# kjenike/panagram

Hardware: AMD Instinct MI355X
Metric: anchored k-mers/sec building pan-kmer bitmap (higher is better)
Workload: dtype u64

## Files before the change

panagram_amd/csrc/pg_anchor.hip:

```cpp
#include "pg_kernels.h"
#include <map>
#include <mutex>
#include <utility>
#include <type_traits>

#include <algorithm>

#ifndef PG_ANCHOR_PART
#define PG_ANCHOR_PART -1
#endif
#define PG_HAS_PART(n) (PG_ANCHOR_PART == -1 || PG_ANCHOR_PART == (n))
#define PG_MAIN_PART (PG_ANCHOR_PART <= 0)
#if defined(PG_PHASE_TIMING) && PG_ANCHOR_PART != -1
#error "a -DPG_PHASE_TIMING build keeps its counters in one device variable: compile pg_anchor.hip as ONE unit (PG_ANCHOR_PART unset)"
#endif

namespace pg {

hipError_t probe_part0(hipStream_t s, uint32_t w, uint32_t ntiles, const SubTable &st, const uint64_t *seqw, const uint32_t *nmw, const uint32_t *has_n,
                       const SeqDesc *sd, const AnchorDesc *ad, const uint32_t *tile_contig, const uint32_t *sched, uint32_t tile_base, uint8_t *out1,
                       uint32_t nbytes, const RowCols &rc, int rowmode, const FuseArgs *fuse);
hipError_t probe_part1(hipStream_t s, uint32_t w, uint32_t ntiles, const SubTable &st, const uint64_t *seqw, const uint32_t *nmw, const uint32_t *has_n,
                       const SeqDesc *sd, const AnchorDesc *ad, const uint32_t *tile_contig, const uint32_t *sched, uint32_t tile_base, uint8_t *out1,
                       uint32_t nbytes, const RowCols &rc, int rowmode, const FuseArgs *fuse);
hipError_t probe_part2(hipStream_t s, uint32_t w, uint32_t ntiles, const SubTable &st, const uint64_t *seqw, const uint32_t *nmw, const uint32_t *has_n,
                       const SeqDesc *sd, const AnchorDesc *ad, const uint32_t *tile_contig, const uint32_t *sched, uint32_t tile_base, uint8_t *out1,
                       uint32_t nbytes, const RowCols &rc, int rowmode, const FuseArgs *fuse);
hipError_t insert_part0(hipStream_t s, uint32_t win, uint32_t ntiles, const SubTable &st, int w, uint32_t bits, uint32_t count_mode, const uint64_t *seqw,
                        const uint32_t *nmw, const uint32_t *has_n, const SeqDesc *sd, const uint32_t *tile0, uint32_t ncontigs,
                        unsigned long long *counters, uint32_t max_probe);
hipError_t insert_part1(hipStream_t s, uint32_t win, uint32_t ntiles, const SubTable &st, int w, uint32_t bits, uint32_t count_mode, const uint64_t *seqw,
                        const uint32_t *nmw, const uint32_t *has_n, const SeqDesc *sd, const uint32_t *tile0, uint32_t ncontigs,
                        unsigned long long *counters, uint32_t max_probe);
hipError_t insert_part2(hipStream_t s, uint32_t win, uint32_t ntiles, const SubTable &st, int w, uint32_t bits, uint32_t count_mode, const uint64_t *seqw,
                        const uint32_t *nmw, const uint32_t *has_n, const SeqDesc *sd, const uint32_t *tile0, uint32_t ncontigs,
                        unsigned long long *counters, uint32_t max_probe);
hipError_t preload_part1();
hipError_t preload_part2();

constexpr int PROBE_SEQW = ((PROBE_TILE + 31) / 32 + 6 + 3) & ~3;
#ifndef PG_ABLATE
#define PG_ABLATE 0
#endif
constexpr uint32_t PROBE_SEQ_BASES = 32u * PROBE_SEQW;
#ifdef PG_PHASE_TIMING
__device__ unsigned long long pg_phase_cycles[1024 * 16];
#define PG_PH_DECL uint32_t ph_acc[12] = {0, 0, 0, 0, 0, 0, 0, 0, 0, 0, 0, 0}; uint32_t ph_t = (uint32_t)__builtin_readcyclecounter();
#define PG_PH(i) { const uint32_t ph_n = (uint32_t)__builtin_readcyclecounter(); ph_acc[i] += ph_n - ph_t; ph_t = ph_n; }
#define PG_PH_FLUSH { if (threadIdx.x == 0) { for (int ph_i = 0; ph_i < 9; ++ph_i) atomicAdd(&pg_phase_cycles[(blockIdx.x & 1023u) * 16u + ph_i], (unsigned long long)ph_acc[ph_i]); atomicAdd(&pg_phase_cycles[(blockIdx.x & 1023u) * 16u + 9], 1ull); atomicAdd(&pg_phase_cycles[(blockIdx.x & 1023u) * 16u + 10], (unsigned long long)ph_acc[10]); } }
#else
#define PG_PH_DECL
#define PG_PH(i)
#define PG_PH_FLUSH
#endif
__device__ __forceinline__ uint64_t revcomp_window(const uint64_t *rw, uint32_t p, uint64_t kmask, uint32_t rcb) {
    return extract_bases32(reinterpret_cast<const uint32_t *>(rw), rcb - p) & kmask;
}

__device__ __forceinline__ void stage_chunk(uint4 *line, uint32_t slot, int slots, const uint4 v) {
    uint2 *const p = reinterpret_cast<uint2 *>(line);
    p[slot] = make_uint2(v.x, v.y);
    p[slots + slot] = make_uint2(v.z, v.w);
}
template <bool TWO, int SLOTS>
__device__ __forceinline__ int scan_line_lds(const uint4 *line, uint64_t key, uint32_t &m0, uint32_t &m1) {
    uint64_t kk[SLOTS];
#pragma unroll
    for (int j = 0; j < SLOTS / 2; ++j) {
        const uint4 v = line[j];
        kk[2 * j] = (uint64_t)v.x | ((uint64_t)v.y << 32);
        kk[2 * j + 1] = (uint64_t)v.z | ((uint64_t)v.w << 32);
    }
    constexpr uint32_t SLOT_BYTES = 8u, MASK0 = 8u * SLOTS;
    m0 = m1 = 0;
    if constexpr (SLOTS == 8) {
        unsigned long long e[8];
#pragma unroll
        for (int sl = 0; sl < 8; ++sl) e[sl] = __builtin_amdgcn_ballot_w64(kk[sl] == key);
        const unsigned long long b0 = e[1] | e[3] | e[5] | e[7], b1 = e[2] | e[3] | e[6] | e[7], b2 = e[4] | e[5] | e[6] | e[7];
        const unsigned long long any = b0 | b1 | b2 | e[0];
        const bool hit = __builtin_amdgcn_inverse_ballot_w64(any);
#if PG_ABLATE == 6
        if (hit) m0 = (uint32_t)b0 | 1u;
        return hit ? 1 : (kk[SLOTS - 1] == EMPTY_KEY ? 0 : -1);
#elif PG_ABLATE == 7
        m0 = (uint32_t)(kk[0] ^ kk[1] ^ kk[2] ^ kk[3] ^ kk[4] ^ kk[5] ^ kk[6] ^ kk[7]) | 1u;
        return (kk[0] ^ kk[3]) == key ? -1 : 1;
#endif
        if (hit) {
            const uint32_t off = (__builtin_amdgcn_inverse_ballot_w64(b0) ? SLOT_BYTES : 0u) | (__builtin_amdgcn_inverse_ballot_w64(b1) ? 2u * SLOT_BYTES : 0u) |
                                 (__builtin_amdgcn_inverse_ballot_w64(b2) ? 4u * SLOT_BYTES : 0u);
            if constexpr (TWO) {
                const uint2 mk = *reinterpret_cast<const uint2 *>(reinterpret_cast<const uint8_t *>(line) + off + MASK0);
                m0 = mk.x;
                m1 = mk.y;
            } else {
                m0 = *reinterpret_cast<const uint32_t *>(reinterpret_cast<const uint8_t *>(line) + off + MASK0);
            }
        }
        return hit ? 1 : (kk[SLOTS - 1] == EMPTY_KEY ? 0 : -1);
    } else {
        int hit = -1;
#pragma unroll
        for (int sl = 0; sl < SLOTS; ++sl) hit = (kk[sl] == key) ? sl : hit;
        if (hit >= 0) {
            const uint2 mk = *reinterpret_cast<const uint2 *>(reinterpret_cast<const uint8_t *>(line) + (uint32_t)hit * SLOT_BYTES + MASK0);
            m0 = mk.x;
            if (TWO) m1 = mk.y;
        }
        return hit >= 0 ? 1 : (kk[SLOTS - 1] == EMPTY_KEY ? 0 : -1);
    }
}


template <bool TWO, int SLOTS>
__device__ __forceinline__ int scan_line_global(const SubTable &st, uint32_t b, uint64_t key, uint32_t &m0, uint32_t &m1) {
    const uint4 *line = reinterpret_cast<const uint4 *>(st.buckets + (uint64_t)b * (16 * SLOTS));
    uint4 v[SLOTS];
#pragma unroll
    for (int sl = 0; sl < SLOTS; ++sl) v[sl] = line[sl];
    m0 = m1 = 0;
#pragma unroll
    for (int sl = 0; sl < SLOTS; ++sl) {
        const uint64_t kk = (uint64_t)v[sl].x | ((uint64_t)v[sl].y << 32);
        const bool hit = (kk == key);
        m0 = hit ? v[sl].z : m0;
        if (TWO) m1 = hit ? v[sl].w : m1;
    }
    const uint64_t last = (uint64_t)v[SLOTS - 1].x | ((uint64_t)v[SLOTS - 1].y << 32);
    return (m0 | m1) ? 1 : (last == EMPTY_KEY ? 0 : -1);
}

template <bool TWO, int SLOTS>
__device__ __forceinline__ void lane_chase(const SubTable &st, uint64_t key, uint32_t level, uint32_t b, uint32_t step,
                                           uint32_t &m0, uint32_t &m1) {
    for (uint64_t n = 0; n < st.nbuckets + GROUP_CHAIN; ++n) {
// ... 260 lines not shown

__device__ __forceinline__ uint32_t lane_up1(uint32_t v) {
    return (uint32_t)__builtin_amdgcn_update_dpp((int)v, (int)v, 0x138 , 0xf, 0xf, false);
}
__device__ __forceinline__ unsigned long long differs_from_lane_below(uint32_t v) {
    uint32_t t;
    asm("s_nop 1\n\tv_xor_b32_dpp %0, %1, %1 wave_shr:1 row_mask:0xf bank_mask:0xf" : "=&v"(t) : "v"(v));
    return __builtin_amdgcn_ballot_w64(t != 0u);
}
#define PG_DPPMIN "s_nop 1\n\tv_min_u32_dpp %0, %0, %1 wave_shr:1 row_mask:0xf bank_mask:0xf\n\t"
template <int W>
__device__ __forceinline__ uint32_t sliding_min(uint32_t x) {
    uint32_t m = x;
    if constexpr (W == 2) asm(PG_DPPMIN : "+v"(m) : "v"(x));
    if constexpr (W == 3) asm(PG_DPPMIN PG_DPPMIN : "+v"(m) : "v"(x));
    if constexpr (W == 4) asm(PG_DPPMIN PG_DPPMIN PG_DPPMIN : "+v"(m) : "v"(x));
    if constexpr (W == 5) asm(PG_DPPMIN PG_DPPMIN PG_DPPMIN PG_DPPMIN : "+v"(m) : "v"(x));
    if constexpr (W == 6) asm(PG_DPPMIN PG_DPPMIN PG_DPPMIN PG_DPPMIN PG_DPPMIN : "+v"(m) : "v"(x));
    if constexpr (W == 7) asm(PG_DPPMIN PG_DPPMIN PG_DPPMIN PG_DPPMIN PG_DPPMIN PG_DPPMIN : "+v"(m) : "v"(x));
    if constexpr (W == 8) asm(PG_DPPMIN PG_DPPMIN PG_DPPMIN PG_DPPMIN PG_DPPMIN PG_DPPMIN PG_DPPMIN : "+v"(m) : "v"(x));
    static_assert(W >= 1 && W <= 8, "minimizer window");
    return m;
}
#undef PG_DPPMIN
__device__ __forceinline__ uint32_t suffix_min8_row(uint32_t x) {
    uint32_t r = x;
    asm("s_nop 1\n\tv_min_u32_dpp %0, %0, %0 row_shl:1 row_mask:0xf bank_mask:0xf\n\t"
        "s_nop 1\n\tv_min_u32_dpp %0, %0, %0 row_shl:2 row_mask:0xf bank_mask:0xf\n\t"
        "s_nop 1\n\tv_min_u32_dpp %0, %0, %0 row_shl:4 row_mask:0xf bank_mask:0xf"
        : "+v"(r));
    return r;
}
#define PG_F "v_min_u32_dpp %0, %0, %0 wave_shr:1 row_mask:0xf bank_mask:0xf\n\t"
#define PG_S(n) "v_min_u32_dpp %1, %1, %1 row_shl:" #n " row_mask:0xf bank_mask:0xf\n\t"
#define PG_N0 "s_nop 0\n\t"
#define PG_N1 "s_nop 1\n\t"
template <int W>
__device__ __forceinline__ uint32_t sliding_min_suffix(uint32_t x, uint32_t &suffix) {
    uint32_t m = x, r = suffix;
    static_assert(W >= 2 && W <= 8, "minimizer window");
    if constexpr (W == 2) asm(PG_N1 PG_F PG_S(1) PG_N1 PG_S(2) PG_N1 PG_S(4) : "+v"(m), "+v"(r));
    if constexpr (W == 3) asm(PG_N1 PG_F PG_S(1) PG_N0 PG_F PG_S(2) PG_N1 PG_S(4) : "+v"(m), "+v"(r));
    if constexpr (W == 4) asm(PG_N1 PG_F PG_S(1) PG_N0 PG_F PG_S(2) PG_N0 PG_F PG_S(4) : "+v"(m), "+v"(r));
    if constexpr (W == 5) asm(PG_N1 PG_F PG_S(1) PG_N0 PG_F PG_S(2) PG_N0 PG_F PG_S(4) PG_N0 PG_F : "+v"(m), "+v"(r));
    if constexpr (W == 6) asm(PG_N1 PG_F PG_S(1) PG_N0 PG_F PG_S(2) PG_N0 PG_F PG_S(4) PG_N0 PG_F PG_N1 PG_F : "+v"(m), "+v"(r));
    if constexpr (W == 7) asm(PG_N1 PG_F PG_S(1) PG_N0 PG_F PG_S(2) PG_N0 PG_F PG_S(4) PG_N0 PG_F PG_N1 PG_F PG_N1 PG_F : "+v"(m), "+v"(r));
    if constexpr (W == 8) asm(PG_N1 PG_F PG_S(1) PG_N0 PG_F PG_S(2) PG_N0 PG_F PG_S(4) PG_N0 PG_F PG_N1 PG_F PG_N1 PG_F PG_N1 PG_F : "+v"(m), "+v"(r));
    suffix = r;
    return m;
}
#undef PG_F
#undef PG_S
#undef PG_N0
#undef PG_N1
__device__ __forceinline__ uint32_t lanes_le_index(unsigned long long mask, uint32_t base) {
    const unsigned long long m1 = mask >> 1;
    const uint32_t c = base + (uint32_t)(mask & 1ull) - 1u;
    return __builtin_amdgcn_mbcnt_hi((uint32_t)(m1 >> 32), __builtin_amdgcn_mbcnt_lo((uint32_t)m1, c));
}

__device__ __forceinline__ uint32_t run_ids(unsigned long long lmask) {
    const uint32_t below = __builtin_amdgcn_mbcnt_hi((uint32_t)(lmask >> 32), __builtin_amdgcn_mbcnt_lo((uint32_t)lmask, ~0u));
    uint32_t rid;
    unsigned long long carry_out;
    asm("v_addc_co_u32_e64 %0, %1, %2, 0, %3" : "=v"(rid), "=s"(carry_out) : "v"(below), "s"(lmask));
    return rid;
}
__device__ __forceinline__ uint32_t set_lane_index(unsigned long long mask, uint32_t base) {
    return __builtin_amdgcn_mbcnt_hi((uint32_t)(mask >> 32), __builtin_amdgcn_mbcnt_lo((uint32_t)mask, base));
}

constexpr int COLS_G = 8;
constexpr uint32_t TILE_SLOTS = PROBE_TILE / 64;
static_assert(PROBE_TILE % 512 == 0, "the column kernels take a tile in units of 512 positions");
__device__ __forceinline__ void cols_or_position(unsigned long long *cols, uint32_t pl, uint32_t m0) {
    while (m0) {
        const uint32_t j = (uint32_t)__ffs((int)m0) - 1u;
        m0 &= m0 - 1u;
        atomicOr(&cols[(pl >> 6) * COLS_G + j], 1ull << (pl & 63u));
    }
}

template <bool TWO, int ROWMODE, int SLOTS, int MAXRUN, bool WIDE, int LEVELS, bool INL = false>
__device__ __forceinline__ void drain_queue(const SubTable &st, uint32_t qn, const uint64_t *sw, const uint64_t *rw, uint32_t *q_line,
                                            uint32_t *q_step, uint16_t *q_pl, uint32_t *lines_w, uint4 *buf,
                                            uint8_t *tile_rows, uint32_t nbytes, const RowCols rc, int lane) {
    const int k = (int)st.k;
    constexpr int LDS_LINE_U4 = SLOTS + 1;
    constexpr int STAGE_ITERS = (MAXRUN * SLOTS + 63) / 64;
    const uint8_t *chunk_base = st.buckets + (uint32_t)(lane % SLOTS) * 16u;
    const uint32_t lbytes = INL ? st.layout * 64u : st.slots * (WIDE ? 8u : 16u);
    static_assert(LEVELS >= 1, "k_probe's entries (home line, group) are turned into (next line, step) by level 1's staged batches");
    for (int level = 1; qn > 0; ++level) {
        __syncthreads();
        if (level > LEVELS) {
            for (uint32_t e = lane; e < qn; e += 64) {
                uint32_t m0, m1;
                const uint64_t key = canonical_from_le(extract_bases(sw, q_pl[e]), k);
                if constexpr (WIDE && INL) {
                    uint32_t rw4[4];
                    lane_chase_inl(st, key, (uint32_t)level, q_line[e], q_step[e], rw4);
                    if (rw4[0] | rw4[1] | rw4[2] | rw4[3]) store_row_regs(tile_rows + (uint64_t)q_pl[e] * nbytes, nbytes, rw4);
                } else if constexpr (WIDE) {
                    lane_chase_wide(st, key, (uint32_t)level, q_line[e], q_step[e], m0, m1);
                    if (m1) store_row_wide(st.masks, st.W, nbytes, tile_rows + (uint64_t)q_pl[e] * nbytes, m0, m1);
                } else {
                    lane_chase<TWO, SLOTS>(st, key, (uint32_t)level, q_line[e], q_step[e], m0, m1);
                    if constexpr (ROWMODE == 3) cols_or_position(reinterpret_cast<unsigned long long *>(tile_rows), q_pl[e], m0);
                    else if (m0 | m1) store_row<ROWMODE>(tile_rows + (uint64_t)q_pl[e] * nbytes, m0, m1, rc);
                }
            }
            break;
        }
        uint32_t kept = 0;
        for (uint32_t i0 = 0; i0 < qn; i0 += 64) {
            const uint32_t e = i0 + lane;
            const bool act = e < qn;
            const uint32_t ec = act ? e : qn - 1;
            uint32_t line = q_line[ec], step = q_step[ec];
            if (GROUP_CHAIN > 1 && level == 1) {
                step = step_of_group(step, st.nbuckets);
                line = next_line(line, step, st.nbuckets);
            }
            const uint32_t pl = q_pl[ec];
            const uint64_t kmask = kmer_mask(k);
            const uint64_t X = extract_bases32(reinterpret_cast<const uint32_t *>(sw), pl) & kmask;
            const uint64_t key = canonical_from_xb(X, revcomp_window(rw, pl, kmask, PROBE_SEQ_BASES - (uint32_t)k), k);
            const uint32_t prev_line = lane_up1(line);
            const bool leader = act && (lane == 0 || line != prev_line);
            const unsigned long long lmask = __builtin_amdgcn_ballot_w64(leader);
            const uint32_t rid = lanes_le_index(lmask, 0u);
            const uint32_t nruns = (uint32_t)__popcll(lmask);
            uint32_t m0 = 0, m1 = 0;
            [[maybe_unused]] uint32_t rw4[4] = {0, 0, 0, 0};
            int rcode = 0;
            const uint32_t padline = lmask ? (uint32_t)__builtin_amdgcn_readlane((int)line, __builtin_ctzll(lmask)) : 0u;
            for (uint32_t r0 = 0; r0 < nruns; r0 += MAXRUN) {
                const uint32_t nl = min((uint32_t)MAXRUN, nruns - r0);
                if (lane < MAXRUN) lines_w[lane] = padline;
                if (leader && rid - r0 < nl) lines_w[rid - r0] = line;
                __syncthreads();
                uint4 v[STAGE_ITERS];
                uint32_t ln[STAGE_ITERS];
#pragma unroll
                for (int u = 0; u < STAGE_ITERS; ++u) ln[u] = lines_w[u * (64 / SLOTS) + lane / SLOTS];
#pragma unroll
                for (int u = 0; u < STAGE_ITERS; ++u) v[u] = *reinterpret_cast<const uint4 *>(chunk_base + (uint64_t)ln[u] * lbytes);
#pragma unroll
                for (int u = 0; u < STAGE_ITERS; ++u) {
                    const uint32_t idx = u * 64 + lane;
                    if constexpr (WIDE) buf[(idx / SLOTS) * LDS_LINE_U4 + (idx % SLOTS)] = v[u];
                    else stage_chunk(buf + (idx / SLOTS) * LDS_LINE_U4, idx % SLOTS, SLOTS, v[u]);
                }
                __syncthreads();
                if (act && rid - r0 < nl) {
                    if constexpr (WIDE && INL) {
                        rcode = scan_keys_inl(buf + (rid - r0) * LDS_LINE_U4, key, st.slots, m1);
                        if (m1) masks_inl(buf + (rid - r0) * LDS_LINE_U4, st.slots, st.W, m1 - 1u, rw4);
                    } else if constexpr (WIDE) {
                        rcode = scan_keys16_lds(buf + (rid - r0) * LDS_LINE_U4, key, m1);
                        m0 = line;
                    } else {
                        rcode = scan_line_lds<TWO, SLOTS>(buf + (rid - r0) * LDS_LINE_U4, key, m0, m1);
                    }
                }
                __syncthreads();
            }
            const bool again = act && rcode < 0;
            if constexpr (WIDE && INL) {
                if (act && m1) store_row_regs(tile_rows + (uint64_t)pl * nbytes, nbytes, rw4);
            } else if constexpr (WIDE) {
                if (act && m1) store_row_wide(st.masks, st.W, nbytes, tile_rows + (uint64_t)pl * nbytes, m0, m1);
            } else {
                if constexpr (ROWMODE == 3) {
                    if (act) cols_or_position(reinterpret_cast<unsigned long long *>(tile_rows), pl, m0);
                } else {
                    if (act && (m0 | m1)) store_row<ROWMODE>(tile_rows + (uint64_t)pl * nbytes, m0, m1, rc);
                }
            }
            const unsigned long long kmask2 = __builtin_amdgcn_ballot_w64(again);
            if (again) {
                const uint32_t slot = set_lane_index(kmask2, kept);
                uint32_t nl2 = line, ns2 = step;
                if constexpr (LEVELS + 1 < (int)GROUP_CHAIN) nl2 = next_line(line, step, st.nbuckets);
                else advance_line(key, (uint32_t)level + 1, st.nbuckets, nl2, ns2);
                q_line[slot] = nl2;
                q_step[slot] = ns2;
                q_pl[slot] = (uint16_t)pl;
            }
            kept += (uint32_t)__popcll(kmask2);
            __syncthreads();
        }
        qn = kept;
    }
}

#ifndef PG_FUSE_LOAD_SC1
#define PG_FUSE_LOAD_SC1 1
#endif
typedef const __attribute__((address_space(1))) uint8_t *GlobalBytes;
template <int NW>
__device__ __forceinline__ void fuse_load_row(GlobalBytes base, uint32_t off, uint32_t (&w)[NW]) {
    GlobalBytes p = base + off;
#if PG_FUSE_LOAD_SC1
#pragma unroll
    for (int i = 0; i + 1 < NW; i += 2) {
        const unsigned long long v = __hip_atomic_load(reinterpret_cast<const __attribute__((address_space(1))) unsigned long long *>(p + 4 * i), __ATOMIC_RELAXED,
                                                       __HIP_MEMORY_SCOPE_AGENT);
        w[i] = (uint32_t)v, w[i + 1] = (uint32_t)(v >> 32);
    }
    if constexpr (NW & 1)
        w[NW - 1] = __hip_atomic_load(reinterpret_cast<const __attribute__((address_space(1))) uint32_t *>(p + 4 * (NW - 1)), __ATOMIC_RELAXED, __HIP_MEMORY_SCOPE_AGENT);
#else
    const WordsN<NW> v = *reinterpret_cast<const __attribute__((address_space(1))) WordsN<NW> *>(p);
#pragma unroll
    for (int i = 0; i < NW; ++i) w[i] = v.w[i];
#endif
}
__device__ __forceinline__ void fuse_flush_word(const uint32_t (&pl)[5], uint32_t *out16, int lane) {
    uint32_t R[16];
#pragma unroll
    for (int q = 0; q < 8; ++q) {
        uint32_t v = 0;
#pragma unroll
        for (int i = 0; i < 5; ++i) v |= ((pl[i] >> q) & 0x01010101u) << i;
        R[2 * q] = v & 0x00FF00FFu;
        R[2 * q + 1] = (v >> 8) & 0x00FF00FFu;
    }
#define PG_XCHG(HALF, BIT)                                                  \
    {                                                                       \
        const bool up = (lane & BIT) != 0;                                  \
        _Pragma("unroll") for (int i = 0; i < HALF; ++i) {                  \
            const uint32_t send = up ? R[i] : R[i + HALF];                  \
            const uint32_t keep = up ? R[i + HALF] : R[i];                  \
            R[i] = keep + (uint32_t)__shfl_xor((int)send, BIT);             \
        }                                                                   \
    }
    PG_XCHG(8, 32)
    PG_XCHG(4, 16)
    PG_XCHG(2, 8)
    PG_XCHG(1, 4)
#undef PG_XCHG
    R[0] += (uint32_t)__shfl_xor((int)R[0], 2);
    R[0] += (uint32_t)__shfl_xor((int)R[0], 1);
    if ((lane & 3) == 0) {
        const uint32_t idx = (uint32_t)lane >> 2;
        out16[(idx >> 1) + ((idx & 1u) ? 8u : 0u)] = R[0];
    }
}
template <int NWP, bool LASTPASS>
__device__ __forceinline__ void tile_statistics_pass(uint32_t *Hc, GlobalBytes rs, uint32_t npos, uint32_t nbytes, uint32_t woff,
                                                     uint32_t keep_last, uint32_t split, uint32_t N, uint32_t (&pcs)[4], uint32_t *cs_out, int lane) {
    const uint32_t N1 = N + 1u;
    uint32_t ones[NWP], twos[NWP], fours[NWP], eights[NWP], sixteens[NWP], hold4[NWP], hold8[NWP];
#pragma unroll
    for (int w = 0; w < NWP; ++w) ones[w] = twos[w] = fours[w] = eights[w] = sixteens[w] = hold4[w] = hold8[w] = 0;
    uint32_t nx[4][NWP];
    auto request = [&](int g, uint32_t (&dst)[4][NWP]) __attribute__((always_inline)) {
#pragma unroll
        for (int i = 0; i < 4; ++i) {
            const uint32_t r = (uint32_t)(4 * g + i) * 64u + (uint32_t)lane;
            fuse_load_row<NWP>(rs, min(r, npos - 1u) * nbytes + woff, dst[i]);
        }
    };
    request(0, nx);
#pragma unroll
    for (int g = 0; g < 4; ++g) {
        uint32_t rw[4][NWP];
#pragma unroll
        for (int i = 0; i < 4; ++i)
#pragma unroll
            for (int w = 0; w < NWP; ++w) rw[i][w] = nx[i][w];
        if (g < 3) request(g + 1, nx);
        uint32_t pc4 = pcs[g];
#pragma unroll
        for (int i = 0; i < 4; ++i) {
// ... 26 lines not shown
            u = twos[w] ^ c2a;
            const uint32_t c4 = (twos[w] & c2a) | (u & c2b);
            twos[w] = u ^ c2b;
            if ((g & 1) == 0) {
                hold4[w] = c4;
            } else {
                u = fours[w] ^ hold4[w];
                const uint32_t c8 = (fours[w] & hold4[w]) | (u & c4);
                fours[w] = u ^ c4;
                if (g == 1) {
                    hold8[w] = c8;
                } else {
                    u = eights[w] ^ hold8[w];
                    sixteens[w] = (eights[w] & hold8[w]) | (u & c8);
                    eights[w] = u ^ c8;
                }
            }
        }
    }
#pragma unroll
    for (int w = 0; w < NWP; ++w) {
        const uint32_t pl[5] = {ones[w], twos[w], fours[w], eights[w], sixteens[w]};
        fuse_flush_word(pl, cs_out + 16 * w, lane);
    }
}

template <int NW>
__device__ __forceinline__ void tile_statistics(uint32_t *H, const uint8_t *tile_rows, uint32_t npos, uint32_t nbytes, const AnchorDesc &a,
                                                uint32_t tile_start, uint32_t tile, const FuseArgs &fo, int lane) {
    const uint32_t N = fo.ngenomes, N1 = N + 1u, hw = fo.hw;
    const uint32_t nh = 2u * N1;
#ifdef PG_PHASE_TIMING
    uint32_t tph[5] = {0, 0, 0, 0, 0}, tph_t = (uint32_t)__builtin_readcyclecounter();
#define PG_TPH(i) { const uint32_t n_ = (uint32_t)__builtin_readcyclecounter(); tph[i] += n_ - tph_t; tph_t = n_; }
#else
#define PG_TPH(i)
#endif
    __builtin_amdgcn_s_waitcnt(0x0F70);
    __syncthreads();
    PG_TPH(0)
    const uint64_t base = reinterpret_cast<uint64_t>(tile_rows);
    GlobalBytes rs = reinterpret_cast<GlobalBytes>(((uint64_t)(uint32_t)__builtin_amdgcn_readfirstlane((int)(uint32_t)(base >> 32)) << 32) |
                                                   (uint32_t)__builtin_amdgcn_readfirstlane((int)(uint32_t)base));
    const uint32_t r100 = (100u - tile_start % 100u) % 100u + 100u * (uint32_t)lane;
    const bool want100 = fo.out100 != nullptr && r100 < npos;
    uint32_t w100[NW];
    fuse_load_row<NW>(rs, min(r100, npos - 1u) * nbytes, w100);
    for (uint32_t i = lane; i < 4u * nh; i += 64) H[i] = 0;
    const uint64_t bin_end = ((uint64_t)(tile_start / a.binlen) + 1u) * a.binlen;
    const uint32_t split = (uint32_t)min((uint64_t)npos, bin_end - tile_start);
    const uint32_t keep = (nbytes & 3u) ? ((1u << (8u * (nbytes & 3u))) - 1u) : ~0u;
    uint32_t *const Hc = H + ((uint32_t)lane & 3u) * nh;
    uint32_t *cs_out = fo.tile_cs + (uint64_t)tile * fo.csw;
    uint32_t pcs[4] = {0, 0, 0, 0};
    __syncthreads();
    PG_TPH(1)
    if constexpr (NW <= 2) {
        tile_statistics_pass<NW, true>(Hc, rs, npos, nbytes, 0u, keep, split, N, pcs, cs_out, lane);
        PG_TPH(2)
    } else {
        tile_statistics_pass<2, false>(Hc, rs, npos, nbytes, 0u, ~0u, split, N, pcs, cs_out, lane);
        PG_TPH(2)
        tile_statistics_pass<NW - 2, true>(Hc, rs, npos, nbytes, 8u, keep, split, N, pcs, cs_out + 32, lane);
    }
    if (want100) {
        uint8_t *dst = fo.out100 + a.out100_off + (uint64_t)((tile_start + r100) / 100u) * nbytes;
#pragma unroll
        for (int i = 0; i < NW; ++i)
#pragma unroll
            for (int b = 0; b < 4; ++b)
                if ((uint32_t)(4 * i + b) < nbytes) dst[4 * i + b] = (uint8_t)(w100[i] >> (8 * b));
    }
    __syncthreads();
    PG_TPH(3)
    uint32_t *th = fo.tile_hist + (uint64_t)tile * hw;
    for (uint32_t i = lane; i < hw; i += 64) {
        const uint32_t lo = H[2u * i] + H[nh + 2u * i] + H[2u * nh + 2u * i] + H[3u * nh + 2u * i];
        const uint32_t hi = H[2u * i + 1u] + H[nh + 2u * i + 1u] + H[2u * nh + 2u * i + 1u] + H[3u * nh + 2u * i + 1u];
        th[i] = lo | (hi << 16);
    }
    PG_TPH(4)
#ifdef PG_PHASE_TIMING
    if (lane == 0)
        for (int i = 0; i < 5; ++i) atomicAdd(&pg_phase_cycles[(blockIdx.x & 1023u) * 16u + 11 + i], (unsigned long long)tph[i]);
#endif
#undef PG_TPH
}

template <bool TWO, int ROWMODE, int SLOTS, bool WIDE>
constexpr bool probe_pipelined = SLOTS == 8 && !WIDE && ROWMODE != 3 && (ROWMODE == 1 || ROWMODE >= 4 || TWO);
template <int W_C, bool TWO, int ROWMODE, int SLOTS, bool M64, bool WIDE = false, bool INL = false, bool FUSE = false>
__global__ __launch_bounds__(64, ((probe_pipelined<TWO, ROWMODE, SLOTS, WIDE> || INL || FUSE) ? 8 : 1))
__attribute__((amdgpu_num_sgpr(80))) void k_probe(const SubTable st, const uint64_t *__restrict__ seqw,
                                              const uint32_t *__restrict__ nmw, const uint32_t *__restrict__ has_n,
                                              const SeqDesc *__restrict__ sd, const AnchorDesc *__restrict__ ad,
                                              const uint32_t *__restrict__ tile_contig,
                                              const uint32_t *__restrict__ sched, uint32_t tile_base,
                                              uint8_t *__restrict__ out1, uint32_t nbytes, const RowCols rc, const FuseArgs fo) {
    constexpr int LDS_LINE_U4 = SLOTS + 1;
    constexpr int MAXRUN = PROBE_MAXRUN;
    constexpr int STAGE_ITERS = (MAXRUN * SLOTS + 63) / 64;
    constexpr int BUF_U4 = ((STAGE_ITERS * 64 + SLOTS - 1) / SLOTS) * LDS_LINE_U4;
    constexpr int OFF_RW = PROBE_SEQW * 8, OFF_NW = OFF_RW + (PROBE_SEQW + 1) * 8, OFF_LW = OFF_NW + PROBE_SEQW * 4;
    constexpr int QCAP = PROBE_QCAP;
    constexpr int OFF_BUF = (OFF_LW + MAXRUN * 4 + 15) & ~15, OFF_QL = OFF_BUF + BUF_U4 * 16, OFF_QS = OFF_QL + QCAP * 4;
    constexpr int OFF_QP = OFF_QS + QCAP * 4, LDS_BYTES = OFF_QP + QCAP * 2;
    static_assert(OFF_LW <= 1020 || PROBE_TILE > 1024, "the sequence words must stay within reach of ds_read2_b32's offsets");
    __shared__ __attribute__((aligned(16))) uint8_t lds[LDS_BYTES];
    uint64_t *const sw = reinterpret_cast<uint64_t *>(lds);
    uint64_t *const rw = reinterpret_cast<uint64_t *>(lds + OFF_RW);
    uint32_t *const nw = reinterpret_cast<uint32_t *>(lds + OFF_NW);
    uint32_t(*const lines_w)[MAXRUN] = reinterpret_cast<uint32_t(*)[MAXRUN]>(lds + OFF_LW);
    uint4(*const buf)[BUF_U4] = reinterpret_cast<uint4(*)[BUF_U4]>(lds + OFF_BUF);
    uint32_t *const q_line = reinterpret_cast<uint32_t *>(lds + OFF_QL);
    uint32_t *const q_step = reinterpret_cast<uint32_t *>(lds + OFF_QS);
    uint16_t *const q_pl = reinterpret_cast<uint16_t *>(lds + OFF_QP);
    PG_PH_DECL
    const int lane = threadIdx.x;
    const int k = (int)st.k;
    if constexpr (W_C != 0) __builtin_assume(k >= 20 && k <= 32);
    const uint32_t tile = sched ? sched[blockIdx.x + tile_base] : blockIdx.x + tile_base;
    const uint32_t c = tile_contig[tile];
    const AnchorDesc a = ad[c];
    const SeqDesc s = sd[c];
    const uint32_t tile_start = (tile - a.tile0) * PROBE_TILE;
    const uint32_t npos = min((uint32_t)PROBE_TILE, a.nkmers - tile_start);
    const bool hasn = has_n[c] != 0;

    for (int i = lane; i < PROBE_SEQW; i += 64) {
        const uint64_t wi = (uint64_t)(tile_start >> 5) + i;
        const uint64_t wv = wi < s.nwords ? seqw[s.seq_off + wi] : 0ull;
        sw[i] = wv;
        rw[PROBE_SEQW - 1 - i] = pair_reverse64(~wv);
        nw[i] = (hasn && wi < s.nwords) ? nmw[s.seq_off + wi] : 0u;
    }
    if (lane == 0) rw[PROBE_SEQW] = 0;
    __syncthreads();

    const uint64_t kmask = W_C ? (((uint64_t)(k == 32 ? ~0u : ((1u << (2 * k - 32)) - 1u)) << 32) | 0xFFFFFFFFull) : kmer_mask(k);
    const uint32_t rcb = PROBE_SEQ_BASES - (uint32_t)k;
    constexpr int HALO = W_C ? W_C - 1 : 0;
    constexpr bool CARRY = W_C >= 2;
    constexpr bool CUT = W_C != 0;
    const uint32_t m = W_C ? (uint32_t)k - W_C + 1 : 0;
    const uint64_t mm64 = (m >= 32) ? ~0ull : ((1ull << (2 * (m ? m : 1))) - 1);
    __shared__ unsigned long long cols[ROWMODE == 3 ? TILE_SLOTS * COLS_G : 1];
    if constexpr (ROWMODE == 3) {
        for (uint32_t i = lane; i < TILE_SLOTS * COLS_G; i += 64) cols[i] = 0;
        __syncthreads();
    }
#if PG_ABLATE == 9 || PG_ABLATE == 10
    uint8_t *tile_rows = out1 + (uint64_t)(blockIdx.x & 255u) * PROBE_TILE * nbytes;
#else
    uint8_t *tile_rows = ROWMODE == 3 ? reinterpret_cast<uint8_t *>(cols) : out1 + a.out_off + (uint64_t)tile_start * nbytes;
#endif
    uint32_t qn = 0;

    const uint8_t *chunk_base = st.buckets + (uint32_t)(lane % SLOTS) * 16u;
    const uint32_t lbytes = INL ? st.layout * 64u : st.slots * (WIDE ? 8u : 16u);

    struct Front {
        uint64_t key;
        uint32_t grp, line, rid, nruns, padline;
        uint32_t adv;
        uint32_t ln[STAGE_ITERS];
        unsigned long long rmask, amask, lmask;
    };
// ... 217 lines not shown
        } else {
            if (ROWMODE == 6 && b0 + (uint32_t)__popcll(f.rmask) < npos) {
                const uint32_t mine = inrange ? m0 : 0u;
                const uint32_t nxt = (uint32_t)__builtin_amdgcn_update_dpp(0, (int)mine, 0x130 , 0xf, 0xf, true);
                struct __attribute__((packed)) U32 { uint32_t v; };
                if (inrange) reinterpret_cast<U32 *>(tile_rows + (uint32_t)pl * 3u)->v = (m0 & 0xFFFFFFu) | (nxt << 24);
            } else if constexpr (ROWMODE == 6) {
                const uint32_t nxt = (uint32_t)__builtin_amdgcn_update_dpp(0, (int)m0, 0x130 , 0xf, 0xf, false);
                const uint32_t o4 = (uint32_t)reinterpret_cast<uintptr_t>(tile_rows) & 3u;
                const uint32_t j = ((uint32_t)pl - o4) & 3u;
                const uint32_t lo = (nxt << 24) | (m0 & 0xFFFFFFu);
                const uint32_t dw = __builtin_amdgcn_alignbit(nxt >> 8, lo, 8u * j);
                const unsigned long long nextin = f.rmask >> 1;
                const unsigned long long dmask = f.rmask & nextin & __builtin_amdgcn_ballot_w64(j != 3u);
                const unsigned long long fmask = f.rmask & (1ull | ~nextin);
                uint8_t *row = tile_rows + (uint32_t)pl * 3u;
                if (__builtin_amdgcn_inverse_ballot_w64(dmask)) *reinterpret_cast<uint32_t *>(row + j) = dw;
                if (__builtin_amdgcn_inverse_ballot_w64(fmask)) store_row<ROWMODE>(row, m0, m1, rc);
            } else
#if PG_ABLATE == 2
            if (inrange && m0 == 0xDEADBEEFu)
#else
            if (ROWMODE == 0 && TWO && rc.words == 3u && nbytes >= 5u && b0 + (uint32_t)__popcll(f.rmask) < npos) {
                const uint32_t mine = inrange ? m0 : 0u;
                const uint32_t nxt = (uint32_t)__builtin_amdgcn_update_dpp(0, (int)mine, 0x130 , 0xf, 0xf, true);
                if (inrange) {
                    typedef uint32_t u32x2u __attribute__((ext_vector_type(2), aligned(1)));
                    const uint32_t t8 = 8u * (nbytes - 4u);
                    u32x2u q = {m0, (m1 & ((1u << t8) - 1u)) | (nxt << t8)};
                    *reinterpret_cast<u32x2u *>(tile_rows + (uint32_t)pl * nbytes) = q;
                }
            } else if (inrange)
#endif
                store_row<ROWMODE>(tile_rows + (ROWMODE == 1 ? (uint32_t)pl : ROWMODE == 4 ? (uint32_t)pl * 4u : ROWMODE == 5 ? (uint32_t)pl * 2u : ROWMODE == 6 ? (uint32_t)pl * 3u : (uint32_t)pl * nbytes), m0, m1, rc);
        }
        PG_PH(6)
    };
    constexpr bool PIPE = probe_pipelined<TWO, ROWMODE, SLOTS, WIDE>;
    constexpr int LEVELS = (W_C >= 6 && !TWO && !WIDE && PROBE_STAGED_LEVELS > 1) ? 1 : PROBE_STAGED_LEVELS;
    static_assert(QCAP >= 128, "an early drain must leave room for a batch");
    constexpr uint32_t QROOM = QCAP - 64;
    uint32_t b0 = 0;
    if constexpr (PIPE) {
        Lines L;
#pragma unroll
        for (int it = 0; it < STAGE_ITERS; ++it) L.v[it] = make_uint4(0, 0, 0, 0);
        PG_PH(0)
        carry = carry_at(0u);
        Front cur = front(0u);
        L = issue(cur, 0u);
        for (;;) {
            PG_PH(7)
            const uint32_t b1 = b0 + cur.adv;
            const bool more = b1 < npos;
            Front nxt = cur;
            __builtin_amdgcn_sched_barrier(0);
            if (more) nxt = front(b1);
            __builtin_amdgcn_sched_barrier(0);
            back(cur, L, b0, [&]() __attribute__((always_inline)) {
                if (more) L = issue(nxt, 0u);
            });
            __builtin_amdgcn_sched_barrier(0);
            b0 = b1;
            if (!more || qn > QROOM) break;
            cur = nxt;
        }
    } else {
        {
            carry = carry_at(0u);
            const Front f = front(0u);
            const Lines L = issue(f, 0u);
            back(f, L, 0u, [] {});
            b0 = f.adv;
        }
        while (b0 < npos && qn <= QROOM) {
            const Front f = front(b0);
            const Lines L = issue(f, 0u);
            back(f, L, b0, [] {});
            b0 += f.adv;
        }
    }
    PG_PH(7)
    for (;;) {
        drain_queue<TWO, ROWMODE, SLOTS, MAXRUN, WIDE, LEVELS, INL>(st, qn, sw, rw, q_line, q_step, q_pl, lines_w[0], buf[0], tile_rows, nbytes, rc, lane);
        qn = 0;
        if (b0 >= npos) break;
        __syncthreads();
        carry = carry_at(b0);
        while (b0 < npos && qn <= QROOM) {
            const Front f = front(b0);
            const Lines L = issue(f, 0u);
            back(f, L, b0, [] {});
            b0 += f.adv;
        }
    }
    PG_PH(8)
    PG_PH_FLUSH
    if constexpr (FUSE) {
        static_assert(ROWMODE != 1 && ROWMODE != 3 && LDS_BYTES >= 4 * 4 * 2 * 129, "fused statistics: rows of 2..16 bytes; four copies of 2 x 129 histogram counters in LDS");
        const AnchorDesc *ad2 = ad;
        const uint32_t *tc2 = tile_contig, *sched2 = sched;
        asm volatile("" : "+s"(ad2), "+s"(tc2), "+s"(sched2));
        const uint32_t tile2 = sched2 ? sched2[blockIdx.x + tile_base] : blockIdx.x + tile_base;
        const AnchorDesc a2 = ad2[tc2[tile2]];
        if (a2.binlen >= (uint32_t)PROBE_TILE) {
            const uint32_t ts2 = (tile2 - a2.tile0) * PROBE_TILE;
            const uint32_t np2 = min((uint32_t)PROBE_TILE, a2.nkmers - ts2);
            const uint8_t *rows2 = out1 + a2.out_off + (uint64_t)ts2 * nbytes;
            uint32_t *H = reinterpret_cast<uint32_t *>(lds);
            if constexpr (WIDE) {
                if (nbytes <= 12u) tile_statistics<3>(H, rows2, np2, nbytes, a2, ts2, tile2, fo, lane);
                else tile_statistics<4>(H, rows2, np2, nbytes, a2, ts2, tile2, fo, lane);
            } else {
                tile_statistics<TWO ? 2 : 1>(H, rows2, np2, nbytes, a2, ts2, tile2, fo, lane);
            }
        }
    }
    if constexpr (ROWMODE == 3) {
        __syncthreads();
        const uint32_t width = nbytes, trel = tile - tile_base;
        unsigned long long *dst = reinterpret_cast<unsigned long long *>(out1) + (uint64_t)trel * TILE_SLOTS * width;
        for (uint32_t i = lane; i < TILE_SLOTS * width; i += 64) dst[i] = cols[(i / width) * COLS_G + i % width];
    }
}

constexpr int INSERT_QCAP = 256;

template <bool COUNT, bool CLAIM = true>
__device__ __forceinline__ int wave_insert_batch(const SubTable &st, bool valid, uint64_t key, uint32_t grp, int w, uint32_t bits,
                                                 uint32_t max_probe, int lane) {
    const uint32_t kstride = key_stride(st), slots = st.slots;
    uint32_t b = home_of_group(grp, st.nbuckets), step = step_of_group(grp, st.nbuckets), probes = 0;
    int s = -1;
    bool done = !valid, fresh = false;
    int r = 0;
    auto shfl64 = [](uint64_t v, int src) __attribute__((always_inline)) {
        return (uint64_t)(uint32_t)__shfl((int)(uint32_t)v, src) | ((uint64_t)(uint32_t)__shfl((int)(uint32_t)(v >> 32), src) << 32);
    };
    auto resolve = [&](uint32_t sl, bool claimed) __attribute__((always_inline)) {
        uint32_t *mp = mask_ptr(st, b, sl, (uint32_t)w);
        if (COUNT) {
            if (*mp < 0xFFFFFF00u) atomicAdd(mp, bits);
        } else if (claimed) {
            *reinterpret_cast<volatile uint32_t *>(mp) = bits;
        } else {
            const uint32_t cur = *mp;
            if ((cur & bits) != bits) *reinterpret_cast<volatile uint32_t *>(mp) = cur | bits;
        }
        r = claimed ? 1 : 0;
        done = true;
    };
    while (__ballot(!done)) {
        if (!done && s >= (int)slots) {
            if (++probes >= max_probe) {
                done = true;
                r = -1;
            } else {
                advance_line(key, probes, st.nbuckets, b, step);
                s = -1;
            }
        }
        if (!done && s < 0) {
            uint8_t *base = st.buckets + (uint64_t)b * line_bytes(st);
            int hit = -1, fr = -1;
            for (uint32_t s0 = 0; s0 < slots; s0 += 8) {
                uint64_t kk[8];
#pragma unroll
// ... 2127 lines not shown
        auto flush = [&]() {
            if (acc) {
                if (is_hist) atomicAdd(&bins[key], (uint32_t)acc);
                else atomicAdd(&colsums[key], acc);
            }
            acc = 0;
        };
#pragma unroll
        for (uint32_t j = 0; j < TR_TILES; ++j) {
            const uint32_t t = t0 + j;
            if (t >= t1) break;
            const uint32_t c = tile_contig[t];
            if (c != cur_c) {
                cur_c = c;
                a = ad[c];
            }
            if (a.binlen < (uint32_t)PROBE_TILE) continue;
            const unsigned long long k2 = is_hist ? (a.bin_off + (uint64_t)(t - a.tile0) * PROBE_TILE / a.binlen + rel) * N1 + pc
                                                  : (unsigned long long)c * N + g;
            if (k2 != key) {
                flush();
                key = k2;
            }
            acc += (v[j] >> shift) & 0xFFFFu;
        }
        flush();
    }
}

hipError_t launch_tile_reduce(hipStream_t st, const FuseArgs &fo, const AnchorDesc *ad, const uint32_t *tile_contig, uint32_t ntiles,
                              uint32_t *bins, unsigned long long *colsums, uint32_t want_colsums) {
    if (ntiles == 0) return hipSuccess;
    const uint32_t nitems = 2u * (fo.ngenomes + 1u) + (want_colsums ? fo.ngenomes : 0u);
    const uint32_t per = std::max(1u, 256u / nitems), groups = (ntiles + TR_TILES - 1) / TR_TILES;
    hipLaunchKernelGGL(k_tile_reduce, dim3((groups + per - 1) / per), dim3(256), 0, st, fo, ad, tile_contig, ntiles, bins, colsums,
                       want_colsums);
    return hipGetLastError();
}

hipError_t launch_window_stats(hipStream_t st, uint32_t ngenomes, const uint8_t *rows, uint64_t nrows, uint32_t nwin,
                               uint32_t pieces, const uint64_t *starts, const uint64_t *ends, unsigned long long *hist,
                               unsigned long long *cs) {
    if (nwin == 0) return hipSuccess;
    hipLaunchKernelGGL(k_window_stats, dim3(nwin, pieces), dim3(256), (2 * ngenomes + 1) * 4, st, ngenomes, rows, nrows,
                       starts, ends, hist, cs);
    return hipGetLastError();
}

hipError_t launch_cols_extract(hipStream_t st, uint32_t ngenomes, const AnchorDesc *ad, const uint32_t *tile_contig,
                               uint32_t tile_base, uint32_t ntiles, const uint8_t *out1, uint32_t g0, uint32_t width, void *dst) {
    if (ntiles == 0 || width == 0) return hipSuccess;
    if (ngenomes <= 8 && g0 < 8)
        hipLaunchKernelGGL(k_cols_extract_b1, dim3((unsigned)(((uint64_t)ntiles + 4 * COLS_TPW - 1) / (4 * COLS_TPW))), dim3(256), 0, st, ngenomes, ad, tile_contig, tile_base,
                           ntiles, out1, g0, width, static_cast<uint8_t *>(dst));
    else
        hipLaunchKernelGGL(k_cols_extract, dim3((unsigned)(((uint64_t)ntiles * TILE_SLOTS + 3) / 4)), dim3(256), 0, st, ngenomes, ad,
                           tile_contig, tile_base, ntiles, out1, g0, width, static_cast<unsigned long long *>(dst));
    return hipGetLastError();
}

hipError_t launch_cols_merge(hipStream_t st, uint32_t ngenomes, const AnchorDesc *ad, const uint32_t *tile_contig,
                             uint32_t tile_base, uint32_t ntiles, uint8_t *out1, const void *src, uint32_t part0,
                             uint32_t nparts, uint64_t part_words, uint32_t per, uint32_t accumulate) {
    if (ntiles == 0 || per == 0 || nparts == 0) return hipSuccess;
    if (ngenomes <= 8)
        hipLaunchKernelGGL(k_cols_merge_b1, dim3((unsigned)(((uint64_t)ntiles + 4 * COLS_TPW - 1) / (4 * COLS_TPW))), dim3(256), 0, st, ngenomes, ad, tile_contig, tile_base,
                           ntiles, out1, static_cast<const uint8_t *>(src), part0, nparts, part_words * 8, per, accumulate);
    else
        hipLaunchKernelGGL(k_cols_merge, dim3((unsigned)(((uint64_t)ntiles * TILE_SLOTS + 3) / 4)), dim3(256), 0, st, ngenomes, ad,
                           tile_contig, tile_base, ntiles, out1, static_cast<const unsigned long long *>(src), part0, nparts,
                           part_words, per, accumulate);
    return hipGetLastError();
}

hipError_t launch_lowres(hipStream_t st, uint32_t ngenomes, const AnchorDesc *ad, const uint32_t *tile_contig,
                         uint32_t ntiles, const uint8_t *out1, uint8_t *outlow, uint32_t step) {
    if (ntiles == 0) return hipSuccess;
    hipLaunchKernelGGL(k_lowres, dim3(ntiles), dim3(64), 0, st, ngenomes, ad, tile_contig, out1, outlow, step);
    return hipGetLastError();
}

#ifdef PG_PHASE_TIMING
}
extern "C" int pg_debug_phase_cycles(unsigned long long *out16, int reset) {
    hipDeviceSynchronize();
    static unsigned long long all[1024 * 16];
    if (hipMemcpyFromSymbol(all, HIP_SYMBOL(pg::pg_phase_cycles), sizeof all) != hipSuccess) return -1;
    for (int i = 0; i < 16; ++i) out16[i] = 0;
    for (int b = 0; b < 1024; ++b)
        for (int i = 0; i < 16; ++i) out16[i] += all[b * 16 + i];
    if (reset) {
        for (auto &x : all) x = 0;
        if (hipMemcpyToSymbol(HIP_SYMBOL(pg::pg_phase_cycles), all, sizeof all) != hipSuccess) return -1;
    }
    return 0;
}
namespace pg {
#endif
hipError_t preload_anchor_kernels() {
    hipFuncAttributes fa;
    hipError_t e = hipFuncGetAttributes(&fa, reinterpret_cast<const void *>(k_lowres));
    if (e == hipSuccess) e = preload_part1();
    if (e == hipSuccess) e = preload_part2();
    return e;
}

hipError_t launch_insert_tiles(hipStream_t s, const SubTable &st, int w, uint32_t bits, int count_mode, const uint64_t *seqw,
                               const uint32_t *nmw, const uint32_t *has_n, const SeqDesc *sd, const uint32_t *tile0,
                               uint32_t ncontigs, uint32_t ntiles, unsigned long long *counters, uint32_t max_probe) {
    if (ntiles == 0) return hipSuccess;
    const uint32_t win = st.m ? st.k - st.m + 1 : 0;
    auto *part = (win == 0 || win == 3 || win == 4) ? insert_part0 : (win == 5 || win == 6) ? insert_part1 : (win == 7 || win == 8) ? insert_part2 : nullptr;
    if (!part) return hipErrorInvalidValue;
    return part(s, win, ntiles, st, w, bits, (uint32_t)count_mode, seqw, nmw, has_n, sd, tile0, ncontigs, counters, max_probe);
}
#endif

}
```

Baseline: 237.6 billion.

## Software-pipeline drain_queue line fetches and drop redundant barriers

Restructures drain_queue's staged levels so that, for non-wide tables, the global fetch of the next batch of bucket lines is issued before scanning the current batch staged in LDS. Two per-iteration __syncthreads are removed. The key computation now uses the caller's kmask and rcb, and run ids come from a ballot-based helper. The level loop is split into a templated first-level/later-level lambda, and phase-timing counters are widened to more slots. The risks are higher register pressure from holding prefetched lines and LDS races now that barriers are gone.

```diff
diff --git a/panagram_amd/csrc/pg_anchor.hip b/panagram_amd/csrc/pg_anchor.hip
--- a/panagram_amd/csrc/pg_anchor.hip
+++ b/panagram_amd/csrc/pg_anchor.hip
@@ -44,14 +44,21 @@
 #endif
 constexpr uint32_t PROBE_SEQ_BASES = 32u * PROBE_SEQW;
 #ifdef PG_PHASE_TIMING
-__device__ unsigned long long pg_phase_cycles[1024 * 16];
-#define PG_PH_DECL uint32_t ph_acc[12] = {0, 0, 0, 0, 0, 0, 0, 0, 0, 0, 0, 0}; uint32_t ph_t = (uint32_t)__builtin_readcyclecounter();
+constexpr uint32_t PG_PH_SLOTS = 32;
+__device__ unsigned long long pg_phase_cycles[1024 * PG_PH_SLOTS];
+#define PG_PH_DECL uint32_t ph_acc[24] = {0, 0, 0, 0, 0, 0, 0, 0, 0, 0, 0, 0, 0, 0, 0, 0, 0, 0, 0, 0, 0, 0, 0, 0}; uint32_t ph_t = (uint32_t)__builtin_readcyclecounter();
 #define PG_PH(i) { const uint32_t ph_n = (uint32_t)__builtin_readcyclecounter(); ph_acc[i] += ph_n - ph_t; ph_t = ph_n; }
-#define PG_PH_FLUSH { if (threadIdx.x == 0) { for (int ph_i = 0; ph_i < 9; ++ph_i) atomicAdd(&pg_phase_cycles[(blockIdx.x & 1023u) * 16u + ph_i], (unsigned long long)ph_acc[ph_i]); atomicAdd(&pg_phase_cycles[(blockIdx.x & 1023u) * 16u + 9], 1ull); atomicAdd(&pg_phase_cycles[(blockIdx.x & 1023u) * 16u + 10], (unsigned long long)ph_acc[10]); } }
+#define PG_PH_COUNT(i, n) { ph_acc[i] += (n); }
+#define PG_PH_FLUSH { if (threadIdx.x == 0) { for (int ph_i = 0; ph_i < 9; ++ph_i) atomicAdd(&pg_phase_cycles[(blockIdx.x & 1023u) * PG_PH_SLOTS + ph_i], (unsigned long long)ph_acc[ph_i]); atomicAdd(&pg_phase_cycles[(blockIdx.x & 1023u) * PG_PH_SLOTS + 9], 1ull); atomicAdd(&pg_phase_cycles[(blockIdx.x & 1023u) * PG_PH_SLOTS + 10], (unsigned long long)ph_acc[10]); for (int ph_i = 16; ph_i < 24; ++ph_i) atomicAdd(&pg_phase_cycles[(blockIdx.x & 1023u) * PG_PH_SLOTS + ph_i], (unsigned long long)ph_acc[ph_i]); } }
+#define PG_PH_PARAMS , uint32_t (&ph_acc)[24], uint32_t &ph_t
+#define PG_PH_ARGS , ph_acc, ph_t
 #else
 #define PG_PH_DECL
 #define PG_PH(i)
+#define PG_PH_COUNT(i, n)
 #define PG_PH_FLUSH
+#define PG_PH_PARAMS
+#define PG_PH_ARGS
 #endif
 __device__ __forceinline__ uint64_t revcomp_window(const uint64_t *rw, uint32_t p, uint64_t kmask, uint32_t rcb) {
     return extract_bases32(reinterpret_cast<const uint32_t *>(rw), rcb - p) & kmask;
@@ -478,77 +485,71 @@
 }
 
 template <bool TWO, int ROWMODE, int SLOTS, int MAXRUN, bool WIDE, int LEVELS, bool INL = false>
-__device__ __forceinline__ void drain_queue(const SubTable &st, uint32_t qn, const uint64_t *sw, const uint64_t *rw, uint32_t *q_line,
-                                            uint32_t *q_step, uint16_t *q_pl, uint32_t *lines_w, uint4 *buf,
-                                            uint8_t *tile_rows, uint32_t nbytes, const RowCols rc, int lane) {
-    const int k = (int)st.k;
+__device__ __forceinline__ void drain_queue(const SubTable &st, uint32_t qn, const uint64_t *sw, const uint64_t *rw, const uint64_t kmask,
+                                            const uint32_t rcb, uint32_t *q_line, uint32_t *q_step, uint16_t *q_pl, uint32_t *lines_w, uint4 *buf,
+                                            uint8_t *tile_rows, uint32_t nbytes, const RowCols rc, int lane PG_PH_PARAMS) {
     constexpr int LDS_LINE_U4 = SLOTS + 1;
     constexpr int STAGE_ITERS = (MAXRUN * SLOTS + 63) / 64;
     const uint8_t *chunk_base = st.buckets + (uint32_t)(lane % SLOTS) * 16u;
     const uint32_t lbytes = INL ? st.layout * 64u : st.slots * (WIDE ? 8u : 16u);
     static_assert(LEVELS >= 1, "k_probe's entries (home line, group) are turned into (next line, step) by level 1's staged batches");
-    for (int level = 1; qn > 0; ++level) {
-        __syncthreads();
-        if (level > LEVELS) {
-            for (uint32_t e = lane; e < qn; e += 64) {
-                uint32_t m0, m1;
-                const uint64_t key = canonical_from_le(extract_bases(sw, q_pl[e]), k);
-                if constexpr (WIDE && INL) {
-                    uint32_t rw4[4];
-                    lane_chase_inl(st, key, (uint32_t)level, q_line[e], q_step[e], rw4);
-                    if (rw4[0] | rw4[1] | rw4[2] | rw4[3]) store_row_regs(tile_rows + (uint64_t)q_pl[e] * nbytes, nbytes, rw4);
-                } else if constexpr (WIDE) {
-                    lane_chase_wide(st, key, (uint32_t)level, q_line[e], q_step[e], m0, m1);
-                    if (m1) store_row_wide(st.masks, st.W, nbytes, tile_rows + (uint64_t)q_pl[e] * nbytes, m0, m1);
-                } else {
-                    lane_chase<TWO, SLOTS>(st, key, (uint32_t)level, q_line[e], q_step[e], m0, m1);
-                    if constexpr (ROWMODE == 3) cols_or_position(reinterpret_cast<unsigned long long *>(tile_rows), q_pl[e], m0);
-                    else if (m0 | m1) store_row<ROWMODE>(tile_rows + (uint64_t)q_pl[e] * nbytes, m0, m1, rc);
-                }
-            }
-            break;
-        }
+    constexpr bool SKEW = !WIDE;
+    auto key_at = [&](const uint32_t pl) __attribute__((always_inline)) {
+        const uint64_t X = extract_bases32(reinterpret_cast<const uint32_t *>(sw), pl) & kmask;
+        const uint64_t B = revcomp_window(rw, pl, kmask, rcb);
+        return ~(X > B ? X : B) & kmask;
+    };
+    PG_PH_COUNT(19, qn)
+    auto staged_level = [&](auto first_c, const uint32_t level) __attribute__((always_inline)) {
+        constexpr bool FIRST = decltype(first_c)::value;
         uint32_t kept = 0;
         for (uint32_t i0 = 0; i0 < qn; i0 += 64) {
             const uint32_t e = i0 + lane;
             const bool act = e < qn;
-            const uint32_t ec = act ? e : qn - 1;
+            const unsigned long long amask = __builtin_amdgcn_ballot_w64(act);
+            const uint32_t ec = min(e, qn - 1u);
             uint32_t line = q_line[ec], step = q_step[ec];
-            if (GROUP_CHAIN > 1 && level == 1) {
+            if constexpr (GROUP_CHAIN > 1 && FIRST) {
                 step = step_of_group(step, st.nbuckets);
                 line = next_line(line, step, st.nbuckets);
             }
             const uint32_t pl = q_pl[ec];
-            const uint64_t kmask = kmer_mask(k);
-            const uint64_t X = extract_bases32(reinterpret_cast<const uint32_t *>(sw), pl) & kmask;
-            const uint64_t key = canonical_from_xb(X, revcomp_window(rw, pl, kmask, PROBE_SEQ_BASES - (uint32_t)k), k);
-            const uint32_t prev_line = lane_up1(line);
-            const bool leader = act && (lane == 0 || line != prev_line);
-            const unsigned long long lmask = __builtin_amdgcn_ballot_w64(leader);
-            const uint32_t rid = lanes_le_index(lmask, 0u);
+            const uint64_t key = key_at(pl);
+            const unsigned long long lmask = amask & (1ull | differs_from_lane_below(line));
+            const bool leader = __builtin_amdgcn_inverse_ballot_w64(lmask);
+            const uint32_t rid = run_ids(lmask);
             const uint32_t nruns = (uint32_t)__popcll(lmask);
             uint32_t m0 = 0, m1 = 0;
             [[maybe_unused]] uint32_t rw4[4] = {0, 0, 0, 0};
             int rcode = 0;
-            const uint32_t padline = lmask ? (uint32_t)__builtin_amdgcn_readlane((int)line, __builtin_ctzll(lmask)) : 0u;
-            for (uint32_t r0 = 0; r0 < nruns; r0 += MAXRUN) {
+            const uint32_t padline = (uint32_t)__builtin_amdgcn_readlane((int)line, 0);
+            uint4 v[STAGE_ITERS];
+            auto fetch = [&](const uint32_t r0) __attribute__((always_inline)) {
                 const uint32_t nl = min((uint32_t)MAXRUN, nruns - r0);
                 if (lane < MAXRUN) lines_w[lane] = padline;
                 if (leader && rid - r0 < nl) lines_w[rid - r0] = line;
                 __syncthreads();
-                uint4 v[STAGE_ITERS];
                 uint32_t ln[STAGE_ITERS];
 #pragma unroll
                 for (int u = 0; u < STAGE_ITERS; ++u) ln[u] = lines_w[u * (64 / SLOTS) + lane / SLOTS];
 #pragma unroll
                 for (int u = 0; u < STAGE_ITERS; ++u) v[u] = *reinterpret_cast<const uint4 *>(chunk_base + (uint64_t)ln[u] * lbytes);
+            };
+            PG_PH_COUNT(20, 1u)
+            if constexpr (SKEW) fetch(0u);
+            for (uint32_t r0 = 0; r0 < nruns; r0 += MAXRUN) {
+                const uint32_t nl = min((uint32_t)MAXRUN, nruns - r0);
+                PG_PH_COUNT(21, 1u)
+                if constexpr (!SKEW) fetch(r0);
+                uint4 *const mine = buf + ((uint32_t)lane / SLOTS) * LDS_LINE_U4;
 #pragma unroll
                 for (int u = 0; u < STAGE_ITERS; ++u) {
-                    const uint32_t idx = u * 64 + lane;
-                    if constexpr (WIDE) buf[(idx / SLOTS) * LDS_LINE_U4 + (idx % SLOTS)] = v[u];
-                    else stage_chunk(buf + (idx / SLOTS) * LDS_LINE_U4, idx % SLOTS, SLOTS, v[u]);
+                    if constexpr (WIDE) mine[u * (64 / SLOTS) * LDS_LINE_U4 + ((uint32_t)lane % SLOTS)] = v[u];
+                    else stage_chunk(mine + u * (64 / SLOTS) * LDS_LINE_U4, (uint32_t)lane % SLOTS, SLOTS, v[u]);
                 }
                 __syncthreads();
+                if constexpr (SKEW)
+                    if (r0 + (uint32_t)MAXRUN < nruns) fetch(r0 + (uint32_t)MAXRUN);
                 if (act && rid - r0 < nl) {
                     if constexpr (WIDE && INL) {
                         rcode = scan_keys_inl(buf + (rid - r0) * LDS_LINE_U4, key, st.slots, m1);
@@ -560,7 +561,6 @@
                         rcode = scan_line_lds<TWO, SLOTS>(buf + (rid - r0) * LDS_LINE_U4, key, m0, m1);
                     }
                 }
-                __syncthreads();
             }
             const bool again = act && rcode < 0;
             if constexpr (WIDE && INL) {
@@ -579,15 +579,46 @@
                 const uint32_t slot = set_lane_index(kmask2, kept);
                 uint32_t nl2 = line, ns2 = step;
                 if constexpr (LEVELS + 1 < (int)GROUP_CHAIN) nl2 = next_line(line, step, st.nbuckets);
-                else advance_line(key, (uint32_t)level + 1, st.nbuckets, nl2, ns2);
+                else advance_line(key, level + 1u, st.nbuckets, nl2, ns2);
                 q_line[slot] = nl2;
                 q_step[slot] = ns2;
                 q_pl[slot] = (uint16_t)pl;
             }
             kept += (uint32_t)__popcll(kmask2);
-            __syncthreads();
-        }
-        qn = kept;
+        }
+        return kept;
+    };
+    for (uint32_t level = 1; qn > 0; ++level) {
+        __syncthreads();
+        if (level > (uint32_t)LEVELS) {
+            PG_PH_COUNT(22, qn)
+            PG_PH_COUNT(23, 1u)
+            for (uint32_t e = lane; e < qn; e += 64) {
+                uint32_t m0, m1;
+                const uint64_t key = key_at(q_pl[e]);
+                if constexpr (WIDE && INL) {
+                    uint32_t rw4[4];
+                    lane_chase_inl(st, key, level, q_line[e], q_step[e], rw4);
+                    if (rw4[0] | rw4[1] | rw4[2] | rw4[3]) store_row_regs(tile_rows + (uint64_t)q_pl[e] * nbytes, nbytes, rw4);
+                } else if constexpr (WIDE) {
+                    lane_chase_wide(st, key, level, q_line[e], q_step[e], m0, m1);
+                    if (m1) store_row_wide(st.masks, st.W, nbytes, tile_rows + (uint64_t)q_pl[e] * nbytes, m0, m1);
+                } else {
+                    lane_chase<TWO, SLOTS>(st, key, level, q_line[e], q_step[e], m0, m1);
+                    if constexpr (ROWMODE == 3) cols_or_position(reinterpret_cast<unsigned long long *>(tile_rows), q_pl[e], m0);
+                    else if (m0 | m1) store_row<ROWMODE>(tile_rows + (uint64_t)q_pl[e] * nbytes, m0, m1, rc);
+                }
+            }
+            PG_PH(18)
+            break;
+        }
+        if (level == 1u) {
+            qn = staged_level(std::true_type{}, level);
+            PG_PH(16)
+        } else if constexpr (LEVELS > 1) {
+            qn = staged_level(std::false_type{}, level);
+            PG_PH(17)
+        }
     }
 }
 
@@ -780,7 +811,7 @@
     PG_TPH(4)
 #ifdef PG_PHASE_TIMING
     if (lane == 0)
-        for (int i = 0; i < 5; ++i) atomicAdd(&pg_phase_cycles[(blockIdx.x & 1023u) * 16u + 11 + i], (unsigned long long)tph[i]);
+        for (int i = 0; i < 5; ++i) atomicAdd(&pg_phase_cycles[(blockIdx.x & 1023u) * PG_PH_SLOTS + 11 + i], (unsigned long long)tph[i]);
 #endif
 #undef PG_TPH
 }
@@ -1164,7 +1195,7 @@
     }
     PG_PH(7)
     for (;;) {
-        drain_queue<TWO, ROWMODE, SLOTS, MAXRUN, WIDE, LEVELS, INL>(st, qn, sw, rw, q_line, q_step, q_pl, lines_w[0], buf[0], tile_rows, nbytes, rc, lane);
+        drain_queue<TWO, ROWMODE, SLOTS, MAXRUN, WIDE, LEVELS, INL>(st, qn, sw, rw, kmask, rcb, q_line, q_step, q_pl, lines_w[0], buf[0], tile_rows, nbytes, rc, lane PG_PH_ARGS);
         qn = 0;
         if (b0 >= npos) break;
         __syncthreads();
@@ -3458,13 +3489,13 @@
 
 #ifdef PG_PHASE_TIMING
 }
-extern "C" int pg_debug_phase_cycles(unsigned long long *out16, int reset) {
+extern "C" int pg_debug_phase_cycles(unsigned long long *out32, int reset) {
     hipDeviceSynchronize();
-    static unsigned long long all[1024 * 16];
+    static unsigned long long all[1024 * pg::PG_PH_SLOTS];
     if (hipMemcpyFromSymbol(all, HIP_SYMBOL(pg::pg_phase_cycles), sizeof all) != hipSuccess) return -1;
-    for (int i = 0; i < 16; ++i) out16[i] = 0;
+    for (uint32_t i = 0; i < pg::PG_PH_SLOTS; ++i) out32[i] = 0;
     for (int b = 0; b < 1024; ++b)
-        for (int i = 0; i < 16; ++i) out16[i] += all[b * 16 + i];
+        for (uint32_t i = 0; i < pg::PG_PH_SLOTS; ++i) out32[i] += all[b * pg::PG_PH_SLOTS + i];
     if (reset) {
         for (auto &x : all) x = 0;
         if (hipMemcpyToSymbol(HIP_SYMBOL(pg::pg_phase_cycles), all, sizeof all) != hipSuccess) return -1;
```

Result: no change. 237.9 billion, median of 6 (+0.1%).
